# npit/video-learning-tf

Measured on AMD Instinct MI355X. Metric: clips/sec (16-frame 227x227) LRCN train step, higher is better.
Workload: dtype f32; 1 GPU; LRCN AlexNet(fc6)+LSTM(256) 16-frame 227x227x3 clips, 101 classes, UCF-101-shaped synthetic, full train step; global_batch=64, clips_per_gpu=64, frames_per_clip=16, parallelism=dp1, optimizer=sgd+clip_by_global_norm(10), init=reference (sigma 0.05), dist_world_size=1

## Files before the change

### include/vltf.h

```cpp
#ifndef VLTF_H
#define VLTF_H

#include <stddef.h>
#include <stdint.h>

#ifdef __cplusplus
extern "C" {
#endif

typedef void* vl_stream_t;
typedef struct vl_conv_desc vl_conv_desc;

typedef struct vl_step_state {
    int64_t step;
    float lr;
    uint32_t tag_origin;
    float adam_lr;
    uint32_t reserved[3];
} vl_step_state;

const char* vl_last_error(void);
int vl_version(void);
int vl_device_count(void);

int vl_input_prep_u8(const uint8_t* src, float* dst, int n, int raw_h, int raw_w, int out_h, int out_w,
                     const int32_t* crop_y, const int32_t* crop_x, const uint8_t* mirror,
                     const float* mean_bgr, int dst_halo, int dst_phase, vl_stream_t stream);
int vl_nhwc_to_nchw(const float* src, float* dst, int n, int h, int w, int c, int dst_halo, int dst_phase, vl_stream_t stream);
int vl_nchw_to_nhwc(const float* src, float* dst, int n, int c, int h, int w, vl_stream_t stream);

int vl_conv_create(vl_conv_desc** out, int cin, int h, int w, int cout, int kh, int kw, int stride, int groups);
void vl_conv_destroy(vl_conv_desc* d);
int vl_conv_out_hw(const vl_conv_desc* d, int* oh, int* ow);
int vl_conv_set_halo(vl_conv_desc* d, int x_halo, int y_halo, int dy_halo, int dx_halo);
int vl_conv_set_x_phase_split(vl_conv_desc* d, int on);
int vl_conv_x_phase(const vl_conv_desc* d);
int vl_set_conv_math(int math);
int vl_conv_math(void);
int vl_conv_set_row_classes(int on);
int vl_conv_fwd(const vl_conv_desc* d, const float* x, const float* w_hwio, const float* bias, float* y,
                int n, int relu, vl_stream_t stream);
int vl_conv_wt_transpose(const vl_conv_desc* d, const float* w_hwio, float* wt, vl_stream_t stream);
int vl_conv_dgrad(const vl_conv_desc* d, const float* dy, const float* wt, float* dx, const float* relu_mask,
                  int n, vl_stream_t stream);
size_t vl_conv_wgrad_ws_bytes(const vl_conv_desc* d, int n);
int vl_conv_wgrad_fuses_bias(const vl_conv_desc* d);
int vl_conv_wgrad(const vl_conv_desc* d, const float* x, const float* dy, float* dw, float* db, void* ws,
                  size_t ws_bytes, int n, vl_stream_t stream);
size_t vl_c8_bytes(int n, int c, int h, int w, int halo);
int vl_pack_c8(const float* x, void* xb, int n, int c, int h, int w, int x_halo, int xb_halo, vl_stream_t stream);
size_t vl_conv_c8_w_bytes(const vl_conv_desc* d, int bwd);
int vl_conv_c8_pack_w(const vl_conv_desc* d, const float* w_hwio, void* wb, int bwd, vl_stream_t stream);
int vl_conv_c8_fwd(vl_conv_desc* d, const void* xb, const void* wb, const float* bias, float* y, void* yb, int n, int relu,
                   vl_stream_t stream);
int vl_conv_c8_dgrad(vl_conv_desc* d, const void* dyb, const void* wbt, float* dx, void* dxb, const float* relu_mask,
                     const void* relu_mask_c8, int n, vl_stream_t stream);
size_t vl_conv_c8_wgrad_ws_bytes(const vl_conv_desc* d, int n);
int vl_conv_c8_wgrad(vl_conv_desc* d, const void* xb, const void* dyb, float* dw, void* ws, size_t ws_bytes, int n,
                     vl_stream_t stream);
int vl_bias_grad_c8(const void* dyb, float* db, float* ws, int n, int c, int h, int w, int halo, vl_stream_t stream);
int vl_pack_kc8(const float* src, void* dst, int64_t positions, int channels, int64_t pos_stride, int64_t ch_stride, vl_stream_t stream);
size_t vl_gemm_kc8_ws_bytes(int m, int n, int k);
int vl_gemm_kc8(const void* a_kc8, const void* b_kc8, float* c, int m, int n, int k, const float* bias, int relu, void* ws,
                size_t ws_bytes, vl_stream_t stream);
int vl_s2d_c8_from_x0(const vl_conv_desc* d, const float* x0, void* xb, int n, vl_stream_t stream);
int vl_input_prep_u8_s2d(const vl_conv_desc* d, const uint8_t* src, void* xb, int n, int raw_h, int raw_w, const int32_t* crop_y,
                         const int32_t* crop_x, const uint8_t* mirror, const float* mean_bgr, vl_stream_t stream);
int vl_s2d_weights(const vl_conv_desc* d, const float* src, float* dst, int grad, vl_stream_t stream);
int vl_bias_grad_nchw(const float* dy, float* db, float* ws, int n, int c, int hw, vl_stream_t stream);

int vl_lrn_fwd(const float* x, float* y, int n, int c, int hw, int radius, float alpha, float beta, float bias,
               vl_stream_t stream);
// ... 109 lines not shown
```

### video-learning-tf_amd/_ffi.py

```python
import ctypes as C
import os

_HERE = os.path.dirname(os.path.abspath(__file__))
LIB_PATH = os.environ.get("VLTF_HIP_LIB") or os.path.join(_HERE, "libvltf_hip.so")

p = C.c_void_p
i32, i64, f32, u32, u64, sz = C.c_int, C.c_int64, C.c_float, C.c_uint32, C.c_uint64, C.c_size_t

SIGNATURES = {
    "vl_last_error": (C.c_char_p, []),
    "vl_version": (i32, []),
    "vl_device_count": (i32, []),
    "vl_input_prep_u8": (i32, [p, p, i32, i32, i32, i32, i32, p, p, p, p, i32, i32, p]),
    "vl_nhwc_to_nchw": (i32, [p, p, i32, i32, i32, i32, i32, i32, p]),
    "vl_nchw_to_nhwc": (i32, [p, p, i32, i32, i32, i32, p]),
    "vl_conv_create": (i32, [C.POINTER(p), i32, i32, i32, i32, i32, i32, i32, i32]),
    "vl_conv_destroy": (None, [p]),
    "vl_conv_out_hw": (i32, [p, C.POINTER(i32), C.POINTER(i32)]),
    "vl_conv_set_halo": (i32, [p, i32, i32, i32, i32]),
    "vl_conv_set_x_phase_split": (i32, [p, i32]),
    "vl_conv_x_phase": (i32, [p]),
    "vl_set_conv_math": (i32, [i32]),
    "vl_conv_math": (i32, []),
    "vl_conv_set_row_classes": (i32, [i32]),
    "vl_gemm_split_ws_bytes": (C.c_size_t, [i32, i32, i32]),
    "vl_conv_fwd": (i32, [p, p, p, p, p, i32, i32, p]),
    "vl_conv_wt_transpose": (i32, [p, p, p, p]),
    "vl_conv_dgrad": (i32, [p, p, p, p, p, i32, p]),
    "vl_conv_wgrad_ws_bytes": (sz, [p, i32]),
    "vl_conv_wgrad_fuses_bias": (i32, [p]),
    "vl_conv_wgrad": (i32, [p, p, p, p, p, p, sz, i32, p]),
    "vl_c8_bytes": (sz, [i32, i32, i32, i32, i32]),
    "vl_pack_c8": (i32, [p, p, i32, i32, i32, i32, i32, i32, p]),
    "vl_conv_c8_w_bytes": (sz, [p, i32]),
    "vl_conv_c8_pack_w": (i32, [p, p, p, i32, p]),
    "vl_conv_c8_fwd": (i32, [p, p, p, p, p, p, i32, i32, p]),
    "vl_conv_c8_dgrad": (i32, [p, p, p, p, p, p, p, i32, p]),
    "vl_pack_kc8": (i32, [p, p, i64, i32, i64, i64, p]),
    "vl_gemm_kc8_ws_bytes": (sz, [i32, i32, i32]),
    "vl_gemm_kc8": (i32, [p, p, p, i32, i32, i32, p, i32, p, sz, p]),
    "vl_s2d_c8_from_x0": (i32, [p, p, p, i32, p]),
    "vl_input_prep_u8_s2d": (i32, [p, p, p, i32, i32, i32, p, p, p, p, p]),
    "vl_s2d_weights": (i32, [p, p, p, i32, p]),
    "vl_bias_grad_c8": (i32, [p, p, p, i32, i32, i32, i32, i32, p]),
    "vl_conv_c8_wgrad_ws_bytes": (sz, [p, i32]),
    "vl_conv_c8_wgrad": (i32, [p, p, p, p, p, sz, i32, p]),
    "vl_bias_grad_nchw": (i32, [p, p, p, i32, i32, i32, p]),
    "vl_lrn_fwd": (i32, [p, p, i32, i32, i32, i32, f32, f32, f32, p]),
    "vl_lrn_bwd": (i32, [p, p, p, i32, i32, i32, i32, f32, f32, f32, i32, i32, i32, p]),
    "vl_lrn_pool_fwd": (i32, [p, p, p, i32, i32, i32, i32, i32, i32, f32, f32, f32, p]),
    "vl_pool_lrn_bwd": (i32, [p, p, p, p, i32, i32, i32, i32, i32, i32, f32, f32, f32, i32, i32, p]),
    "vl_pool_lrn_bwd_test_ranges": (i32, [i32]),
    "vl_lrn_pool_fwd_c8": (i32, [p, i32, p, p, i32, i32, i32, i32, i32, i32, f32, f32, f32, p]),
    "vl_pool_lrn_bwd_c8": (i32, [p, i32, p, p, p, i32, i32, i32, i32, i32, i32, f32, f32, f32, i32, i32, p]),
    "vl_maxpool_fwd": (i32, [p, p, p, i32, i32, i32, i32, i32, i32, i64, i64, i64, i64, p]),
    "vl_maxpool_bwd": (i32, [p, p, p, p, i32, i32, i32, i32, i32, i32, i64, i64, i64, i64, i32, p]),
    "vl_gemm": (i32, [i32, i32, i32, i32, i32, p, i64, p, i64, p, i64, p, i32, p, p, sz, p]),
# ... 88 lines not shown
```

### video-learning-tf_amd/csrc/conv_desc.h

```cpp
#pragma once
#include <hip/hip_runtime.h>
#include <stdint.h>

struct vl_conv_rowcls {
    int ncls;
    int oh0[5];
    int rows[5];
    int K[5];
    int tab0[5];
    int rt0[5];
};

struct vl_conv_desc {
    int cin, h, w, cout, kh, kw, stride, groups;
    int oh, ow, pt, pl, pb, pr;
    int cig, cog;
    int K;
    int Kd;
    int x_halo, y_halo, dy_halo, dx_halo;
    int x_phase;
    int2* ktab2_fwd;
    int* ktab_fwd;
    int2* ptab2_fwd;
    int2* ptab2_bwd;
    int* ptab_fwd;
    int* ptab_bwd;
    int* rowtab_fwd;
    int* rowtab_bwd;
    int fwd_padded, bwd_padded;
    vl_conv_rowcls rc_fwd, rc_bwd;
    uint32_t* wsplit_fwd;
    uint32_t* wsplit_bwd;
    int* c8_toff_fwd;
    int* c8_toff_bwd;
};

void conv_c8_free_tables(vl_conv_desc* d);
int conv_c8_build_tables(vl_conv_desc* d);
```

### video-learning-tf_amd/csrc/mfma_gemm.hip

```cpp
#include <stdlib.h>
#include <string.h>

#include "common.h"
#include "conv_desc.h"

typedef float f32x16 __attribute__((ext_vector_type(16)));
typedef const __attribute__((address_space(4))) int* const_int_ptr;
__device__ __forceinline__ const_int_ptr as_const(const int* p) { return (const_int_ptr)(uintptr_t)p; }
static constexpr int NT = 256;
static constexpr int KBLK = 16;

static constexpr uint32_t OOB_OFF = 0xF0000000u;
static constexpr int64_t MAX_BUF_BYTES = 0xE0000000ll;

__device__ __forceinline__ __amdgpu_buffer_rsrc_t make_rsrc(const float* base, int64_t bytes) {
    return __builtin_amdgcn_make_buffer_rsrc(const_cast<float*>(base), 0, (int)(uint32_t)bytes, 0x00020000);
}
__device__ __forceinline__ float buf_load(__amdgpu_buffer_rsrc_t r, uint32_t voff, int soff) {
    return __builtin_bit_cast(float, __builtin_amdgcn_raw_buffer_load_b32(r, (int)voff, soff, 0));
}

template <int BX, int BR>
struct LdsTile {
    static constexpr int STR = BR + 2;
// ... 557 lines not shown

template <int I> struct IntC { static constexpr int value = I; };
template <int B, int E, typename F>
__device__ __forceinline__ void static_for(F&& f) {
    if constexpr (B < E) {
        f(IntC<B>{});
        static_for<B + 1, E>(f);
    }
}
struct SplitBf16 {
    i32x4 p[3];
};
template <int NPC>
__device__ __forceinline__ void split_pieces(float x0, float x1, int (&out)[3]) {
    f32x2 r = {x0, x1};
#pragma unroll
    for (int k = 0; k < NPC; ++k) {
        const uint32_t h = __builtin_bit_cast(uint32_t, __builtin_convertvector(r, bf16x2));
        out[k] = (int)h;
        if (k + 1 < NPC) r = f32x2{r[0] - __uint_as_float(h << 16), r[1] - __uint_as_float(h & 0xffff0000u)};
    }
}
__device__ constexpr int kProdA[6] = {0, 0, 1, 1, 0, 2};
__device__ constexpr int kProdB[6] = {0, 1, 0, 1, 2, 0};
constexpr int split_products(int math) { return math == 6 ? 6 : math == 3 ? 3 : 1; }
constexpr int split_pieces_of(int math) { return math == 6 ? 3 : math == 3 ? 2 : 1; }
__device__ __forceinline__ f32x16 mfma_bf16(const i32x4& a, const i32x4& b, const f32x16& c) {
    return __builtin_amdgcn_mfma_f32_32x32x16_bf16(__builtin_bit_cast(bf16x8, a), __builtin_bit_cast(bf16x8, b), c, 0, 0, 0);
}

template <int BN, int WM, int WN, int MATH = 0, bool X4 = false>
__global__ __launch_bounds__(NT, 1) void wgrad_dma_kernel(const ConvGeom g, const DyParams d, const EpiRowMajor::Params pe,
                                                          int tiles_i, int tiles_j, int groups, int units, int rtiles,
                                                          int rt_per_split, float* db_slabs, int db_stride) {
    using C = WgradDmaCfg<BN>;
    constexpr int BM = C::BM, STR = C::STR, SA = BM * STR, BUF = C::BUF;
    constexpr int TM = BM / WM / 32, TN = BN / WN / 32;
    constexpr int RA = BM / 4, RB = BN / 4;
    static_assert(WM * WN == 4 && TM * WM * 32 == BM && TN * WN * 32 == BN, "tile shape");
    static_assert(RA + RB <= 10 * 2 * TM * TN, "row fetches must leave the last third of a tile's MFMAs to cover their latency");
    static_assert(!X4 || (MATH != 0 && BN == 128 && BM == 128), "the 16-byte fetch form: split-product modes, 128 x 128 tiles");
    constexpr int GSTR = 258, SA4 = 32 * GSTR, BUF4 = 64 * GSTR;
    extern __shared__ __attribute__((aligned(16))) float ldsw[];

    const int tiles = tiles_i * tiles_j;
    const int k8 = blockIdx.x >> 3;
    const int unit = (k8 / tiles) * 8 + (blockIdx.x & 7);
    if (unit >= units) return;
    const int tile_id = k8 % tiles;
    const int ti_blk = tile_id % tiles_i, tj_blk = tile_id / tiles_i;
    const int zg = unit % groups, zs = unit / groups;
    const int i0 = ti_blk * BM, j0 = tj_blk * BN;
    const int lane = threadIdx.x & 63;
    const int wave = __builtin_amdgcn_readfirstlane(threadIdx.x >> 6);
    const int wi0 = (wave / WN) * (BM / WM), wj0 = (wave % WN) * (BN / WN);

    const i32x4 rs_x = rsrc_words(g.x + (int64_t)zg * g.grp_stride, (g.total - (int64_t)zg * g.grp_stride) * 4);
    const int64_t goff = (int64_t)zg * d.Cog * d.plane;
    const i32x4 rs_dy = rsrc_words(d.dy + goff, (d.total - goff) * 4);
    const int* tab = g.ktab + i0 + wave * RA;
    const uint32_t lds0 = (uint32_t)(uintptr_t)(__attribute__((address_space(3))) float*)ldsw;
    const int row_bytes = (int)(d.plane * 4);
    const int b_row0 = j0 + wave * RB;
    const int b_last = d.Cog - 1;
    const int64_t dy_img = (int64_t)d.Cout_total * d.plane;

    uint32_t voff_x, voff_dy;
    auto decode = [&](int rt) __attribute__((always_inline)) {
        const int m = X4 ? rt * 64 + 4 * (lane & 15) : rt * 64 + lane;
        const bool vm = m < g.M;
        const uint32_t mm = vm ? m : 0;
        const uint32_t n = fd_div(mm, g.dOHW);
        const uint32_t p = mm - n * g.OHW;
        const uint32_t oh = fd_div(p, g.dOW);
        const uint32_t ow = p - oh * g.OW;
        const int ih0 = (int)oh * g.stride - g.pt + g.halo, iw0 = (int)ow * g.col_mul + g.col_add;
        const uint32_t vx = (uint32_t)((int64_t)n * g.img_stride + (int64_t)ih0 * g.Wp + iw0) * 4u;
        const uint32_t vd = (uint32_t)((int64_t)n * dy_img + (int64_t)(oh + d.halo) * d.OWp + ow + d.halo) * 4u;
        voff_x = vm ? vx : OOB_OFF;
        voff_dy = vm ? vd : OOB_OFF;
        asm volatile("" : "+v"(voff_x), "+v"(voff_dy));
    };
    int tabv[RA];
    auto load_table = [&](int rt) __attribute__((always_inline)) {
        const const_int_ptr tt = (const_int_ptr)(uintptr_t)(tab + rt * g.zero);
#pragma unroll
        for (int f = 0; f < RA; ++f) tabv[f] = tt[f];
    };
    auto pin_table = [&]() __attribute__((always_inline)) {
#pragma unroll
        for (int f = 0; f < RA; ++f) asm volatile("" : "+s"(tabv[f]));
    };
    auto dma = [&](const int nb, const int f, int rt_next) __attribute__((always_inline)) {
        const int z = rt_next * g.zero;
        if (f < RA) {
            const uint32_t la = lds0 + (uint32_t)(wave * (RA * STR) + z) * 4u;
            lds_dma_row(rs_x, la + (uint32_t)(nb * BUF + f * STR) * 4u, voff_x, tabv[f]);
        } else {
            const int r = f - RA;
            const uint32_t lb = lds0 + (uint32_t)(SA + wave * (RB * STR) + z) * 4u;
            lds_dma_row(rs_dy, lb + (uint32_t)(nb * BUF + r * STR) * 4u, voff_dy, min(b_row0 + z + r, b_last) * row_bytes);
        }
    };
    uint32_t vrow_a[8], vrow_b[8];
    if constexpr (X4) {
#pragma unroll
        for (int j = 0; j < 8; ++j) {
            const int rl = wave * 8 + j + 32 * (lane >> 4);
            vrow_a[j] = i0 + rl < g.K ? (uint32_t)g.ktab[i0 + rl] : OOB_OFF;
            vrow_b[j] = j0 + rl < d.Cog ? (uint32_t)(j0 + rl) * (uint32_t)row_bytes : OOB_OFF;
        }
    }
    auto dma_x4 = [&](const int nb, const int f, int rt_next) __attribute__((always_inline)) {
        const int z = rt_next * g.zero;
        if (f < 8) {
            const uint32_t vo = (vrow_a[f] == OOB_OFF || voff_x == OOB_OFF) ? OOB_OFF : vrow_a[f] + voff_x;
            lds_dma_row4(rs_x, lds0 + (uint32_t)(nb * BUF4 + (wave * 8 + f) * GSTR + z) * 4u, vo, 0);
        } else {
            const uint32_t vo = (vrow_b[f - 8] == OOB_OFF || voff_dy == OOB_OFF) ? OOB_OFF : vrow_b[f - 8] + voff_dy;
            lds_dma_row4(rs_dy, lds0 + (uint32_t)(nb * BUF4 + SA4 + (wave * 8 + f - 8) * GSTR + z) * 4u, vo, 0);
        }
    };
    const int ones_row = (db_slabs != nullptr && g.K >= i0 && g.K < i0 + BM) ? g.K - i0 : -1;
    auto finish_tile = [&](const int nb) __attribute__((always_inline)) {
        asm volatile("s_waitcnt vmcnt(0)" ::: "memory");
        if constexpr (X4) {
            if (ones_row >= 0 && ((ones_row & 31) >> 3) == wave) ldsw[nb * BUF4 + (ones_row & 31) * GSTR + (ones_row >> 5) * 64 + lane] = 1.0f;
        } else {
            if (ones_row >= 0 && (ones_row / RA) == wave) ldsw[nb * BUF + ones_row * STR + lane] = 1.0f;
        }
        __syncthreads();
    };

    f32x16 acc[TM][TN];
#pragma unroll
    for (int a = 0; a < TM; ++a)
#pragma unroll
        for (int b = 0; b < TN; ++b)
#pragma unroll
            for (int q = 0; q < 16; ++q) acc[a][b][q] = 0.f;

    const int rt0 = zs * rt_per_split;
    const int rt1 = min(rtiles, rt0 + rt_per_split);
    const int ntiles = rt1 - rt0;
    if (ntiles > 0) {
        decode(rt0);
        load_table(rt0);
        pin_table();
        if constexpr (X4) {
#pragma unroll
            for (int f = 0; f < 16; ++f) dma_x4(0, f, rt0);
        } else {
#pragma unroll
            for (int f = 0; f < RA + RB; ++f) dma(0, f, rt0);
        }
        decode(rt0 + 1);
        finish_tile(0);
    }
    const float* fa = ldsw + (wi0 + (lane & 31)) * STR + 2 * (lane >> 5);
    const float* fb = ldsw + SA + (wj0 + (lane & 31)) * STR + 2 * (lane >> 5);

    auto tile = [&](const int cur, int rt_next) __attribute__((always_inline)) {
        float2 af[2][TM], bf[2][TN];
#pragma unroll
        for (int a = 0; a < TM; ++a) af[0][a] = *reinterpret_cast<const float2*>(fa + cur * BUF + a * 32 * STR);
#pragma unroll
        for (int b = 0; b < TN; ++b) bf[0][b] = *reinterpret_cast<const float2*>(fb + cur * BUF + b * 32 * STR);
#pragma unroll
        for (int t = 0; t < 16; ++t) {
            const int c = t & 1, nx = c ^ 1;
            if (t + 1 < 16) {
#pragma unroll
                for (int a = 0; a < TM; ++a) af[nx][a] = *reinterpret_cast<const float2*>(fa + cur * BUF + a * 32 * STR + 4 * (t + 1));
#pragma unroll
                for (int b = 0; b < TN; ++b) bf[nx][b] = *reinterpret_cast<const float2*>(fb + cur * BUF + b * 32 * STR + 4 * (t + 1));
            }
#pragma unroll
            for (int m = 0; m < 2 * TM * TN; ++m) {
                const int a = (m % (TM * TN)) / TN, b = m % TN;
                if (m < TM * TN) acc[a][b] = __builtin_amdgcn_mfma_f32_32x32x2f32(af[c][a].x, bf[c][b].x, acc[a][b], 0, 0, 0);
                else acc[a][b] = __builtin_amdgcn_mfma_f32_32x32x2f32(af[c][a].y, bf[c][b].y, acc[a][b], 0, 0, 0);
                const int f = t * (2 * TM * TN) + m;
                if (f < RA + RB) {
                    dma(cur ^ 1, f, rt_next);
                    __builtin_amdgcn_sched_barrier(0);
                }
            }
            if (t == 10) {
                load_table(rt_next + 1);
                __builtin_amdgcn_sched_barrier(0);
            }
            if (t == 13) {
                int rtn = rt_next + 1;
                asm volatile("" : "+s"(rtn));
                decode(rtn);
                pin_table();
                __builtin_amdgcn_sched_barrier(0);
            }
        }
        finish_tile(cur ^ 1);
    };
    const float* fa3 = ldsw + (wi0 + (lane & 31)) * STR + 8 * (lane >> 5);
    const float* fb3 = ldsw + SA + (wj0 + (lane & 31)) * STR + 8 * (lane >> 5);
    auto tile_split = [&](const int cur, int rt_next) __attribute__((always_inline)) {
        constexpr int NP = split_products(MATH), NPC = split_pieces_of(MATH);
        constexpr int NMS = NP * TM * TN, NTOT = 4 * NMS, NF = X4 ? 16 : RA + RB;
        constexpr int FSPAN = NTOT >= 28 ? NTOT - 14 : NTOT / 2;
        constexpr int FPM = (NF + FSPAN - 1) / FSPAN, FEND = (NF + FPM - 1) / FPM;
        constexpr int LT = FEND > NTOT - 12 ? FEND : NTOT - 12;
        constexpr int PIN = LT + 2 > NTOT - 6 ? LT + 2 : NTOT - 6;
        static_assert(PIN < NTOT, "the tile must leave room to load and pin the next table");
        SplitBf16 As[2][TM], Bs[2][TN];
        auto load_split = [&](const int st, SplitBf16 (&A)[TM], SplitBf16 (&B)[TN]) __attribute__((always_inline)) {
#pragma unroll
            for (int a = 0; a < TM; ++a)
#pragma unroll
                for (int q = 0; q < 4; ++q) {
                    const float2 v = X4 ? *reinterpret_cast<const float2*>(ldsw + cur * BUF4 + (lane & 31) * GSTR + (wi0 / 32 + a) * 64 + 16 * st +
                                                                            8 * (lane >> 5) + 2 * q)
                                        : *reinterpret_cast<const float2*>(fa3 + cur * BUF + a * 32 * STR + 16 * st + 2 * q);
                    int pc[3] = {0, 0, 0};
                    split_pieces<NPC>(v.x, v.y, pc);
#pragma unroll
                    for (int k = 0; k < NPC; ++k) A[a].p[k][q] = pc[k];
                }
#pragma unroll
            for (int b = 0; b < TN; ++b)
#pragma unroll
                for (int q = 0; q < 4; ++q) {
                    const float2 v = X4 ? *reinterpret_cast<const float2*>(ldsw + cur * BUF4 + SA4 + (lane & 31) * GSTR + (wj0 / 32 + b) * 64 +
                                                                            16 * st + 8 * (lane >> 5) + 2 * q)
                                        : *reinterpret_cast<const float2*>(fb3 + cur * BUF + b * 32 * STR + 16 * st + 2 * q);
                    int pc[3] = {0, 0, 0};
// ... 9 lines not shown
            static_for<0, NMS>([&](auto MI) __attribute__((always_inline)) {
                constexpr int m = decltype(MI)::value;
                constexpr int prod = m / (TM * TN), a = (m % (TM * TN)) / TN, b = m % TN;
                acc[a][b] = mfma_bf16(As[c][a].p[kProdA[prod]], Bs[c][b].p[kProdB[prod]], acc[a][b]);
                constexpr int idx = st * NMS + m;
                static_for<0, FPM>([&](auto EI) __attribute__((always_inline)) {
                    constexpr int f = idx * FPM + decltype(EI)::value;
                    if constexpr (f < NF) {
                        if constexpr (X4) dma_x4(cur ^ 1, f, rt_next);
                        else dma(cur ^ 1, f, rt_next);
                    }
                });
                __builtin_amdgcn_sched_barrier(0x106);
                if constexpr (idx == LT) load_table(rt_next + 1);
                if constexpr (idx == PIN) {
                    int rtn = rt_next + 1;
                    asm volatile("" : "+s"(rtn));
                    decode(rtn);
                    pin_table();
                }
            });
        });
        finish_tile(cur ^ 1);
    };
    auto run_tile = [&](const int cur, int rt_next) __attribute__((always_inline)) {
        if constexpr (MATH != 0) tile_split(cur, rt_next);
        else tile(cur, rt_next);
    };
    int rt = rt0;
    for (int i = 0; i + 1 < ntiles; i += 2, rt += 2) {
        run_tile(0, rt + 1);
        run_tile(1, rt + 2);
    }
    if (ntiles > 0 && (ntiles & 1)) run_tile(0, rt + 1);

    EpiRowMajor::template apply<TM, TN>(pe, zg, zs, i0 + wi0, j0 + wj0, acc);
    if (ones_row >= 0) {
        float* dbs = db_slabs + (int64_t)zs * db_stride + zg * d.Cog;
        const int lr = ones_row - wi0;
        if (lr >= 0 && lr < BM / WM) {
            const int a = lr >> 5, rr = lr & 31;
            const int q = (rr & 3) + 4 * (rr >> 3);
            if (((rr >> 2) & 1) == (lane >> 5)) {
#pragma unroll
                for (int b = 0; b < TN; ++b) {
                    const int j = j0 + wj0 + 32 * b + (lane & 31);
                    float v = 0.f;
#pragma unroll
                    for (int aa = 0; aa < TM; ++aa)
#pragma unroll
                        for (int qq = 0; qq < 16; ++qq)
                            if (aa == a && qq == q) v = acc[aa][b][qq];
                    if (j < d.Cog) dbs[j] = v;
                }
            }
        }
    }
}

typedef float f32x4 __attribute__((ext_vector_type(4)));
typedef float f32x4u __attribute__((ext_vector_type(4), aligned(4)));

struct ConvDmaParams {
    const float* w;
    int64_t w_ld;
    int64_t w_grp_stride;
    int64_t w_bytes;
// ... 798 lines not shown
        const int blocks = (int)((count + 255) / 256 < 4096 ? (count + 255) / 256 : 4096);
        hipLaunchKernelGGL(reduce_slabs_kernel<1>, dim3(blocks), dim3(256), 0, s, ws, out, count, splits, slab_stride, bias, ncols, ldc, relu, mask);
    }
}

static const bool kConvStaged = vl_exp_env("VL_CONV_STAGED") != nullptr;
static const bool kGemmNoSplit = vl_exp_env("VL_GEMM_NOSPLIT") != nullptr;
static const bool kConvNoWideStore = vl_exp_env("VL_CONV_NO_WIDE_STORE") != nullptr;
static const bool kConvNoTailSplit = vl_exp_env("VL_CONV_NO_TAIL_SPLIT") != nullptr;
static const bool kConvNoLoadPick = vl_exp_env("VL_CONV_NO_LOAD_PICK") != nullptr;
static const bool kWgradDword = vl_exp_env("VL_WGRAD_DWORD") != nullptr;
static const bool kRing8 = vl_exp_env("VL_CONV_RING8") != nullptr;

static int g_conv_math = [] {
    const char* e = vl_exp_env("VL_CONV_MATH");
    return e == nullptr ? 0 : strcmp(e, "bf16x3") == 0 ? 3 : strcmp(e, "bf16x6") == 0 ? 6 : strcmp(e, "bf16") == 0 ? 1 : 0;
}();

extern "C" int vl_set_conv_math(int math) {
    VL_CHECK(math == 0 || math == 1 || math == 3 || math == 6, "vl_set_conv_math: 0 (fp32), 1 (bf16), 3 (bf16x3) or 6 (bf16x6)");
    g_conv_math = math;
    return 0;
}

extern "C" int vl_conv_math(void) { return g_conv_math; }

static int g_conv_row_classes = 1;

extern "C" int vl_conv_set_row_classes(int on) {
    g_conv_row_classes = on ? 1 : 0;
    return 0;
}


static void tf_same_pad(int in, int k, int s, int* out, int* before, int* after) {
    *out = (in + s - 1) / s;
    int total = (*out - 1) * s + k - in;
    if (total < 0) total = 0;
    *before = total / 2;
    *after = total - *before;
}


static void k_to_row(int k, int kh, int kw, int cg, bool permuted, int* ky, int* kx, int* c) {
    if (permuted) {
        const int cl = k % KBLK, t = k / KBLK;
        *kx = t % kw;
        *ky = (t / kw) % kh;
        *c = (t / (kw * kh)) * KBLK + cl;
    } else {
        *c = k % cg;
        *kx = (k / cg) % kw;
        *ky = k / (cg * kw);
    }
}

static void free_dev(void* p) {
    if (p) (void)hipFree(p);
}

template <class T>
static int upload(T** dev, const T* host, size_t count) {
    free_dev(*dev);
    *dev = nullptr;
    hipError_t e = hipMalloc((void**)dev, sizeof(T) * count);
    if (e == hipSuccess) e = hipMemcpy(*dev, host, sizeof(T) * count, hipMemcpyHostToDevice);
// ... 62 lines not shown
            }
        for (int i = 0; i < ncls; ++i) {
            const int c = order[i], Kc = (c_hi[c] - c_lo[c] + 1) * kw * cg;
            rc->oh0[i] = c_oh0[c]; rc->rows[i] = c_rows[c]; rc->K[i] = Kc;
            if (Kc == K) {
                rc->tab0[i] = 0; rc->rt0[i] = 0;
                continue;
            }
            rc->tab0[i] = (int)n1; rc->rt0[i] = (int)n3;
            int kc = 0;
            for (int k = 0; k < K; ++k) {
                int ky, kx, ch;
                k_to_row(k, kh, kw, cg, true, &ky, &kx, &ch);
                if (ky < c_lo[c] || ky > c_hi[c]) continue;
                h1[n1 + kc] = h1[k];
                if (kc % KBLK == 0) h3[n3 + kc / KBLK] = h3[k / KBLK];
                ++kc;
            }
            n1 += ((Kc + 127) / 128) * 128 + 256;
            n3 += (((Kc + 127) / 128) * 128 + 256) / KBLK;
        }
        rc->ncls = ncls;
    }
    int rcode = upload(dev1, h1, n1);
    if (rcode == 0) rcode = upload(dev2, h2, pad);
    if (rcode == 0 && rowtab) rcode = upload(rowtab, h3, n3);
    if (rcode && rc) rc->ncls = 0;
    free(h1);
    free(h2);
    free(h3);
    return rcode;
}

static int rebuild_tables(vl_conv_desc* d) {
    d->fwd_padded = d->x_halo >= d->pt && d->x_halo >= d->pb && d->x_halo >= d->pl && d->x_halo >= d->pr;
    if (!d->fwd_padded) d->x_phase = 1;
    const int ph = d->x_phase > 1 ? d->x_phase : 1, shift = d->x_halo - d->pl;
    int rc = build_ktabs(&d->ktab_fwd, &d->ktab2_fwd, nullptr, d->kh, d->kw, d->cig, d->h, d->w, d->x_halo, false, ph, shift);
    if (rc == 0)
        rc = build_ktabs(&d->ptab_fwd, &d->ptab2_fwd, &d->rowtab_fwd, d->kh, d->kw, d->cig, d->h, d->w, d->x_halo, d->cig % KBLK == 0, ph,
                         shift, d->stride == 1 ? &d->rc_fwd : nullptr, d->pt, d->oh);
    if (rc == 0 && d->stride == 1) {
        rc = build_ktabs(&d->ptab_bwd, &d->ptab2_bwd, &d->rowtab_bwd, d->kh, d->kw, d->cog, d->oh, d->ow, d->dy_halo, d->cog % KBLK == 0, 1,
                         0, &d->rc_bwd, d->kh - 1 - d->pt, d->h);
        const int need = (d->kh - 1 - d->pt > d->pt ? d->kh - 1 - d->pt : d->pt);
        const int needw = (d->kw - 1 - d->pl > d->pl ? d->kw - 1 - d->pl : d->pl);
        d->bwd_padded = d->dy_halo >= need && d->dy_halo >= needw;
    }
    if (rc == 0) rc = conv_c8_build_tables(d);
    return rc;
}

extern "C" int vl_conv_create(vl_conv_desc** out, int cin, int h, int w, int cout, int kh, int kw, int stride, int groups) {
    VL_CHECK(out, "vl_conv_create: null out");
    VL_CHECK(cin > 0 && cout > 0 && h > 0 && w > 0 && kh > 0 && kw > 0 && stride > 0 && groups > 0, "vl_conv_create: bad geometry");
    VL_CHECK(cin % groups == 0 && cout % groups == 0, "vl_conv_create: channels not divisible by groups");
    VL_CHECK(h < 0x4000 && w < 0x4000 && kh < 256 && kw < 256, "vl_conv_create: plane too large");
    vl_conv_desc* d = (vl_conv_desc*)calloc(1, sizeof(vl_conv_desc));
    VL_CHECK(d, "vl_conv_create: out of host memory");
    d->cin = cin; d->h = h; d->w = w; d->cout = cout; d->kh = kh; d->kw = kw; d->stride = stride; d->groups = groups;
    tf_same_pad(h, kh, stride, &d->oh, &d->pt, &d->pb);
    tf_same_pad(w, kw, stride, &d->ow, &d->pl, &d->pr);
    d->cig = cin / groups;
    d->cog = cout / groups;
    d->K = kh * kw * d->cig;
    d->Kd = kh * kw * d->cog;
    const size_t sf = (size_t)groups * ceil_div(d->K, KBLK) * 24 * (ceil_div(d->cog, 128) * 128) * 4;
    const size_t sb = (size_t)groups * ceil_div(d->Kd, KBLK) * 24 * (ceil_div(d->cig, 128) * 128) * 4;
    const bool images = sf <= (64u << 20) && sb <= (64u << 20);
    if (rebuild_tables(d) || (images && (hipMalloc((void**)&d->wsplit_fwd, sf) != hipSuccess || hipMalloc((void**)&d->wsplit_bwd, sb) != hipSuccess))) {
        vl_conv_destroy(d);
        vl_set_error("vl_conv_create: device table allocation failed");
        return 2;
    }
    *out = d;
    return 0;
}

extern "C" int vl_conv_set_halo(vl_conv_desc* d, int x_halo, int y_halo, int dy_halo, int dx_halo) {
    VL_CHECK(d, "vl_conv_set_halo: null descriptor");
    VL_CHECK(x_halo >= 0 && y_halo >= 0 && dy_halo >= 0 && dx_halo >= 0 && x_halo < 64 && y_halo < 64 && dy_halo < 64 && dx_halo < 64,
             "vl_conv_set_halo: bad halo");
    d->x_halo = x_halo; d->y_halo = y_halo; d->dy_halo = dy_halo; d->dx_halo = dx_halo;
    VL_CHECK(rebuild_tables(d) == 0, "vl_conv_set_halo: device table allocation failed");
    return 0;
}

extern "C" int vl_conv_set_x_phase_split(vl_conv_desc* d, int on) {
    VL_CHECK(d, "vl_conv_set_x_phase_split: null descriptor");
    VL_CHECK(!on || d->fwd_padded, "vl_conv_set_x_phase_split: needs the padded x layout (set the halo first)");
    d->x_phase = (on && d->stride > 1) ? d->stride : 1;
    VL_CHECK(rebuild_tables(d) == 0, "vl_conv_set_x_phase_split: device table allocation failed");
    return 0;
}

extern "C" int vl_conv_x_phase(const vl_conv_desc* d) { return d && d->x_phase > 1 ? d->x_phase : 1; }

extern "C" void vl_conv_destroy(vl_conv_desc* d) {
    if (!d) return;
    free_dev(d->ktab_fwd);
    free_dev(d->ktab2_fwd);
    free_dev(d->ptab_fwd);
    free_dev(d->ptab2_fwd);
    free_dev(d->ptab_bwd);
    free_dev(d->ptab2_bwd);
    free_dev(d->rowtab_fwd);
    free_dev(d->rowtab_bwd);
    free_dev(d->wsplit_fwd);
    free_dev(d->wsplit_bwd);
    conv_c8_free_tables(d);
    free(d);
}

extern "C" int vl_conv_out_hw(const vl_conv_desc* d, int* oh, int* ow) {
    VL_CHECK(d, "vl_conv_out_hw: null descriptor");
    if (oh) *oh = d->oh;
    if (ow) *ow = d->ow;
    return 0;
}

struct ConvOut {
    float* y;
    const float* bias;
    const float* mask;
    int relu;
    int y_halo, m_halo, OH, OW;
};

template <int BM, int WM, int WN, bool PADDED>
static int launch_conv(const ConvGeom& g, const float* w, int64_t w_ld, int w_grp_stride, const int* row_tab, int Cog,
                       int Cout_total, const ConvOut& o, hipStream_t s) {
    constexpr int BN = 128, BR = KBLK;
    using LA = ConvWeightKX<BM, BR>;
    using LB = ConvGather<BN, BR, PADDED>;
    typename LA::Params pa{w, w_ld, Cog, g.K, (int64_t)w_grp_stride, row_tab};
    EpiConvNCHW::Params pe;
    pe.y = o.y; pe.bias = o.bias; pe.mask = o.mask; pe.relu = o.relu;
    pe.Cog = Cog; pe.Cout_total = Cout_total; pe.OHW = g.OHW; pe.OW = g.OW; pe.M = g.M;
    pe.dOHW = g.dOHW; pe.dOW = g.dOW;
    pe.y_halo = o.y_halo; pe.y_wp = o.OW + 2 * o.y_halo; pe.y_plane = (int64_t)(o.OH + 2 * o.y_halo) * pe.y_wp;
// ... 534 lines not shown
                       ceil_div(rtiles, splits));
    VL_LAUNCH_CHECK();
    return reduce_wgrad(d, dw, ws, splits, s);
}

template <int BN, int WM, int WN>
static int launch_wgrad_dma(const vl_conv_desc* d, const ConvGeom& g, const float* dy, float* dw, float* db, float* ws, int splits,
                            hipStream_t s) {
    using C = WgradDmaCfg<BN>;
    DyParams pb;
    dy_params(d, g, dy, pb);
    const int64_t slab = (int64_t)d->K * d->cout;
    EpiRowMajor::Params pe{splits > 1 ? ws : dw, d->cout, d->K, d->cog, nullptr, nullptr, 0, d->cog, splits > 1 ? slab : 0};
    const int tiles_i = ceil_div(d->K, C::BM), tiles_j = ceil_div(d->cog, BN);
    const int rtiles = ceil_div(g.M, C::BR);
    static bool attr_set[8] = {false, false, false, false, false, false, false, false};
    int v = g_conv_math == 6 ? 3 : g_conv_math == 3 ? 2 : g_conv_math == 1 ? 1 : 0;
    auto kern = v == 3 ? wgrad_dma_kernel<BN, WM, WN, 6> : v == 2 ? wgrad_dma_kernel<BN, WM, WN, 3>
              : v == 1 ? wgrad_dma_kernel<BN, WM, WN, 1> : wgrad_dma_kernel<BN, WM, WN, 0>;
    if constexpr (BN == 128) {
        if (v != 0 && g.OW % 4 == 0 && g.col_mul == 1 && !kWgradDword) {
            kern = v == 3 ? wgrad_dma_kernel<BN, WM, WN, 6, true> : v == 2 ? wgrad_dma_kernel<BN, WM, WN, 3, true> : wgrad_dma_kernel<BN, WM, WN, 1, true>;
            v += 4;
        }
    }
    if (!attr_set[v]) {
        VL_HIP(hipFuncSetAttribute(reinterpret_cast<const void*>(kern), hipFuncAttributeMaxDynamicSharedMemorySize, (int)C::LDS_BYTES));
        attr_set[v] = true;
    }
    float* db_slabs = db ? (splits > 1 ? ws + (int64_t)splits * slab : db) : nullptr;
    const int units = d->groups * splits;
    dim3 grid((unsigned)(ceil_div(units, 8) * 8 * tiles_i * tiles_j), 1, 1);
    hipLaunchKernelGGL(kern, grid, dim3(NT), C::LDS_BYTES, s, g, pb, pe, tiles_i, tiles_j, d->groups, units, rtiles,
                       ceil_div(rtiles, splits), db_slabs, d->cout);
    VL_LAUNCH_CHECK();
    if (db && splits > 1) {
        launch_reduce_slabs(s, db_slabs, db, (int64_t)d->cout, splits, (int64_t)d->cout, nullptr, 0, 0, 0, nullptr);
        VL_LAUNCH_CHECK();
    }
    return reduce_wgrad(d, dw, ws, splits, s);
}

static int device_cus() {
    static int cus = 0;
    if (!cus) {
        int dev = 0;
        hipDeviceProp_t p;
        if (hipGetDevice(&dev) == hipSuccess && hipGetDeviceProperties(&p, dev) == hipSuccess) cus = p.multiProcessorCount;
        if (cus <= 0) cus = 256;
    }
    return cus;
}

static int wgrad_splits(const vl_conv_desc* d, int n) {
    const int64_t M = (int64_t)n * d->oh * d->ow;
    const int tiles = ceil_div(d->K, 128) * ceil_div(d->cog, d->cog % 128 == 0 ? 128 : 96) * d->groups;
    if (!d->fwd_padded) {
        const int rtiles = ceil_div(M, 32);
        int splits = ceil_div(2048, tiles);
        return splits > rtiles ? rtiles : (splits < 1 ? 1 : splits);
    }
    const int rtiles = ceil_div(M, 64);
    static const int forced = vl_exp_env("VL_WGRAD_SPLITS") ? atoi(vl_exp_env("VL_WGRAD_SPLITS")) : 0;
    if (forced >= 1 && forced <= rtiles) return forced;
    const int per_xcd = device_cus() / 8 > 0 ? device_cus() / 8 : 1;
    const int64_t slab_bytes = ((int64_t)d->K + 1) * d->cout * 4;
    int best = 1;
// ... 333 lines not shown
```

### video-learning-tf_amd/ops.py

```python
import ctypes as C

import torch

from . import _ffi

F32 = torch.float32


def stream():
    return torch.cuda.current_stream().cuda_stream


def _p(t):
    return None if t is None else t.data_ptr()


def _f32(*ts):
    for t in ts:
        if t is None:
            continue
        if not (t.is_cuda and t.dtype == F32):
            raise _ffi.VltfError("expected a CUDA/HIP float32 tensor, got %s on %s" % (t.dtype, t.device))


# ... 578 lines not shown
              stream())


def step_guard(skip, *lstm_workspaces):
    _skip_word(skip)
    first = True
    for ws in lstm_workspaces:
        if ws is not None:
            _ffi.call("vl_status_or", _p(skip), _p(ws), int(first), stream())
            first = False
    return skip


def fill(t, value):
    _f32(t)
    _ffi.call("vl_fill", _p(t), t.numel(), value, stream())


CONV_MATH = {"f32": 0, "bf16": 1, "bf16x3": 3, "bf16x6": 6}


def set_conv_math(name):
    if name not in CONV_MATH:
        raise _ffi.VltfError("conv math must be one of %s, not %r" % (sorted(CONV_MATH), name))
    _ffi.call("vl_set_conv_math", CONV_MATH[name])


def conv_math():
    return {v: k for k, v in CONV_MATH.items()}[int(_ffi.lib().vl_conv_math())]


def conv_set_row_classes(on=True):
    _ffi.call("vl_conv_set_row_classes", int(bool(on)))


def relu_grad(d, y, count=None):
    _f32(d, y); _dense(d, y)
    _ffi.call("vl_relu_grad", _p(d), _p(y), d.numel() if count is None else int(count), stream())


def copy2d(src, dst, rows, cols, src_ld=None, dst_ld=None):
    _f32(src, dst)
    _ffi.call("vl_copy2d", _p(src), cols if src_ld is None else int(src_ld), _p(dst), cols if dst_ld is None else int(dst_ld),
              int(rows), int(cols), stream())


ELTWISE_OP = {"add": 0, "avg": 1, "maximum": 2}


def eltwise2(a, b, out, op, count=None):
    _f32(a, b, out)
    _ffi.call("vl_eltwise2", _p(a), _p(b), _p(out), a.numel() if count is None else int(count), ELTWISE_OP[op], stream())


def max2_grad(a, b, d, da, db, count=None):
    _f32(a, b, d, da, db)
    _ffi.call("vl_max2_grad", _p(a), _p(b), _p(d), _p(da), _p(db), a.numel() if count is None else int(count), stream())


FUSE_OP = {"avg": 0, "maximum": 1}


def _ptr_list(ts):
    arr = (C.c_void_p * len(ts))()
    for i, t in enumerate(ts):
        arr[i] = None if t is None else t.data_ptr()
# ... 56 lines not shown
```

Baseline: 1906 clips/s.

## Skip MFMA k-steps in conv wgrad for padding-only output windows

Precomputes, for each 128-row weight-gradient tile of padded stride-1 convolutions, the output-pixel window that can touch real input. In the f32 wgrad DMA kernel, a wave ballot marks 4-pixel k-steps whose pixels all fall outside that window, and inline-asm branches skip those MFMA groups. Padded taps then stop doing zero multiplies at border pixels. The cost is extra scalar branching, hand-written asm with manual nops, and accumulator fences before the epilogue. The path is on by default and only applies in the plain f32 math mode.

```diff
diff --git a/include/vltf.h b/include/vltf.h
--- a/include/vltf.h
+++ b/include/vltf.h
@@ -38,6 +38,7 @@
 int vl_set_conv_math(int math);
 int vl_conv_math(void);
 int vl_conv_set_row_classes(int on);
+int vl_conv_set_wgrad_skip(int on);
 int vl_conv_fwd(const vl_conv_desc* d, const float* x, const float* w_hwio, const float* bias, float* y,
                 int n, int relu, vl_stream_t stream);
 int vl_conv_wt_transpose(const vl_conv_desc* d, const float* w_hwio, float* wt, vl_stream_t stream);
diff --git a/video-learning-tf_amd/_ffi.py b/video-learning-tf_amd/_ffi.py
--- a/video-learning-tf_amd/_ffi.py
+++ b/video-learning-tf_amd/_ffi.py
@@ -23,6 +23,7 @@
     "vl_set_conv_math": (i32, [i32]),
     "vl_conv_math": (i32, []),
     "vl_conv_set_row_classes": (i32, [i32]),
+    "vl_conv_set_wgrad_skip": (i32, [i32]),
     "vl_gemm_split_ws_bytes": (C.c_size_t, [i32, i32, i32]),
     "vl_conv_fwd": (i32, [p, p, p, p, p, i32, i32, p]),
     "vl_conv_wt_transpose": (i32, [p, p, p, p]),
diff --git a/video-learning-tf_amd/csrc/conv_desc.h b/video-learning-tf_amd/csrc/conv_desc.h
--- a/video-learning-tf_amd/csrc/conv_desc.h
+++ b/video-learning-tf_amd/csrc/conv_desc.h
@@ -27,6 +27,7 @@
     int* ptab_bwd;
     int* rowtab_fwd;
     int* rowtab_bwd;
+    int* wgrad_win;
     int fwd_padded, bwd_padded;
     vl_conv_rowcls rc_fwd, rc_bwd;
     uint32_t* wsplit_fwd;
diff --git a/video-learning-tf_amd/csrc/mfma_gemm.hip b/video-learning-tf_amd/csrc/mfma_gemm.hip
--- a/video-learning-tf_amd/csrc/mfma_gemm.hip
+++ b/video-learning-tf_amd/csrc/mfma_gemm.hip
@@ -613,8 +613,9 @@
 template <int BN, int WM, int WN, int MATH = 0, bool X4 = false>
 __global__ __launch_bounds__(NT, 1) void wgrad_dma_kernel(const ConvGeom g, const DyParams d, const EpiRowMajor::Params pe,
                                                           int tiles_i, int tiles_j, int groups, int units, int rtiles,
-                                                          int rt_per_split, float* db_slabs, int db_stride) {
+                                                          int rt_per_split, float* db_slabs, int db_stride, const int* win) {
     using C = WgradDmaCfg<BN>;
+    constexpr bool SKIP = MATH == 0 && !X4;
     constexpr int BM = C::BM, STR = C::STR, SA = BM * STR, BUF = C::BUF;
     constexpr int TM = BM / WM / 32, TN = BN / WN / 32;
     constexpr int RA = BM / 4, RB = BN / 4;
@@ -646,6 +647,16 @@
     const int b_last = d.Cog - 1;
     const int64_t dy_img = (int64_t)d.Cout_total * d.plane;
 
+    uint32_t w_oh_lo = 0, w_oh_span = 0, w_ow_lo = 0, w_ow_span = 0, w_on = 0;
+    if constexpr (SKIP) {
+        if (win != nullptr) {
+            const const_int_ptr wp = (const_int_ptr)(uintptr_t)(win + 4 * ti_blk);
+            w_oh_lo = (uint32_t)wp[0]; w_oh_span = (uint32_t)wp[1]; w_ow_lo = (uint32_t)wp[2]; w_ow_span = (uint32_t)wp[3];
+            w_on = wp[1] >= 0 ? 1u : 0u;
+        }
+        asm volatile("" : "+v"(w_oh_lo), "+v"(w_oh_span), "+v"(w_ow_lo), "+v"(w_ow_span), "+v"(w_on));
+    }
+    uint64_t skipq = 0;
     uint32_t voff_x, voff_dy;
     auto decode = [&](int rt) __attribute__((always_inline)) {
         const int m = X4 ? rt * 64 + 4 * (lane & 15) : rt * 64 + lane;
@@ -661,6 +672,18 @@
         voff_x = vm ? vx : OOB_OFF;
         voff_dy = vm ? vd : OOB_OFF;
         asm volatile("" : "+v"(voff_x), "+v"(voff_dy));
+        if constexpr (SKIP) {
+            const bool outside = !vm || oh - w_oh_lo > w_oh_span || ow - w_ow_lo > w_ow_span;
+            uint64_t b = __builtin_amdgcn_ballot_w64(outside && w_on != 0);
+            b &= b >> 1;
+            b &= b >> 2;
+            b &= 0x1111111111111111ull;
+            b = (b | b >> 3) & 0x0303030303030303ull;
+            b = (b | b >> 6) & 0x000f000f000f000full;
+            b = (b | b >> 12) & 0x000000ff000000ffull;
+            b = (b | b >> 24) & 0xffffull;
+            skipq = (skipq & 0xffffffffull) | b << 32;
+        }
     };
     int tabv[RA];
     auto load_table = [&](int rt) __attribute__((always_inline)) {
@@ -726,6 +749,7 @@
     const int ntiles = rt1 - rt0;
     if (ntiles > 0) {
         decode(rt0);
+        skipq >>= 16;
         load_table(rt0);
         pin_table();
         if constexpr (X4) {
@@ -736,50 +760,88 @@
             for (int f = 0; f < RA + RB; ++f) dma(0, f, rt0);
         }
         decode(rt0 + 1);
+        skipq >>= 16;
         finish_tile(0);
     }
     const float* fa = ldsw + (wi0 + (lane & 31)) * STR + 2 * (lane >> 5);
     const float* fb = ldsw + SA + (wj0 + (lane & 31)) * STR + 2 * (lane >> 5);
 
+    auto mfma1 = [](f32x16& cacc, float x, float y, uint64_t sq, auto T, bool first) __attribute__((always_inline)) {
+        constexpr int t = decltype(T)::value;
+        if (first) asm volatile("s_nop 1\n\ts_bitcmp1_b64 %3, %4\n\ts_cbranch_scc1 1f\n\tv_mfma_f32_32x32x2_f32 %0, %1, %2, %0\n1:"
+                                : "+a"(cacc) : "v"(x), "v"(y), "s"(sq), "n"(t) : "scc");
+        else asm volatile("s_bitcmp1_b64 %3, %4\n\ts_cbranch_scc1 1f\n\tv_mfma_f32_32x32x2_f32 %0, %1, %2, %0\n1:"
+                          : "+a"(cacc) : "v"(x), "v"(y), "s"(sq), "n"(t) : "scc");
+    };
+    auto mfma_step = [](f32x16 (&cacc)[TM][TN], const float2 (&A)[TM], const float2 (&B)[TN], uint64_t sq, auto T) __attribute__((always_inline)) {
+        constexpr int t = decltype(T)::value;
+        if constexpr (TM == 2 && TN == 2) {
+            asm volatile("s_bitcmp1_b64 %12, %13\n\ts_cbranch_scc1 1f\n\t"
+                         "v_mfma_f32_32x32x2_f32 %0, %4, %8, %0\n\tv_mfma_f32_32x32x2_f32 %1, %4, %10, %1\n\t"
+                         "v_mfma_f32_32x32x2_f32 %2, %6, %8, %2\n\tv_mfma_f32_32x32x2_f32 %3, %6, %10, %3\n\t"
+                         "v_mfma_f32_32x32x2_f32 %0, %5, %9, %0\n\tv_mfma_f32_32x32x2_f32 %1, %5, %11, %1\n\t"
+                         "v_mfma_f32_32x32x2_f32 %2, %7, %9, %2\n\tv_mfma_f32_32x32x2_f32 %3, %7, %11, %3\n1:"
+                         : "+a"(cacc[0][0]), "+a"(cacc[0][1]), "+a"(cacc[1][0]), "+a"(cacc[1][1])
+                         : "v"(A[0].x), "v"(A[0].y), "v"(A[1].x), "v"(A[1].y), "v"(B[0].x), "v"(B[0].y), "v"(B[1].x), "v"(B[1].y), "s"(sq), "n"(t)
+                         : "scc");
+        } else {
+            static_assert(TM == 1 && TN == 3, "mfma_step: wave tile shapes of launch_wgrad_dma");
+            asm volatile("s_bitcmp1_b64 %11, %12\n\ts_cbranch_scc1 1f\n\t"
+                         "v_mfma_f32_32x32x2_f32 %0, %3, %5, %0\n\tv_mfma_f32_32x32x2_f32 %1, %3, %7, %1\n\tv_mfma_f32_32x32x2_f32 %2, %3, %9, %2\n\t"
+                         "v_mfma_f32_32x32x2_f32 %0, %4, %6, %0\n\tv_mfma_f32_32x32x2_f32 %1, %4, %8, %1\n\tv_mfma_f32_32x32x2_f32 %2, %4, %10, %2\n1:"
+                         : "+a"(cacc[0][0]), "+a"(cacc[0][1]), "+a"(cacc[0][2])
+                         : "v"(A[0].x), "v"(A[0].y), "v"(B[0].x), "v"(B[0].y), "v"(B[1].x), "v"(B[1].y), "v"(B[2].x), "v"(B[2].y), "s"(sq), "n"(t)
+                         : "scc");
+        }
+    };
+    auto acc_fence = [&]() __attribute__((always_inline)) {
+#pragma unroll
+        for (int k = 0; k < TM * TN; ++k) asm volatile("s_nop 7\n\ts_nop 7\n\ts_nop 7" : "+a"(acc[k / TN][k % TN]));
+    };
     auto tile = [&](const int cur, int rt_next) __attribute__((always_inline)) {
         float2 af[2][TM], bf[2][TN];
 #pragma unroll
         for (int a = 0; a < TM; ++a) af[0][a] = *reinterpret_cast<const float2*>(fa + cur * BUF + a * 32 * STR);
 #pragma unroll
         for (int b = 0; b < TN; ++b) bf[0][b] = *reinterpret_cast<const float2*>(fb + cur * BUF + b * 32 * STR);
-#pragma unroll
-        for (int t = 0; t < 16; ++t) {
-            const int c = t & 1, nx = c ^ 1;
-            if (t + 1 < 16) {
+        static_for<0, 16>([&](auto T) __attribute__((always_inline)) {
+            constexpr int t = decltype(T)::value;
+            constexpr int c = t & 1, nx = c ^ 1;
+            if constexpr (t + 1 < 16) {
 #pragma unroll
                 for (int a = 0; a < TM; ++a) af[nx][a] = *reinterpret_cast<const float2*>(fa + cur * BUF + a * 32 * STR + 4 * (t + 1));
 #pragma unroll
                 for (int b = 0; b < TN; ++b) bf[nx][b] = *reinterpret_cast<const float2*>(fb + cur * BUF + b * 32 * STR + 4 * (t + 1));
             }
-#pragma unroll
-            for (int m = 0; m < 2 * TM * TN; ++m) {
-                const int a = (m % (TM * TN)) / TN, b = m % TN;
-                if (m < TM * TN) acc[a][b] = __builtin_amdgcn_mfma_f32_32x32x2f32(af[c][a].x, bf[c][b].x, acc[a][b], 0, 0, 0);
-                else acc[a][b] = __builtin_amdgcn_mfma_f32_32x32x2f32(af[c][a].y, bf[c][b].y, acc[a][b], 0, 0, 0);
-                const int f = t * (2 * TM * TN) + m;
-                if (f < RA + RB) {
-                    dma(cur ^ 1, f, rt_next);
-                    __builtin_amdgcn_sched_barrier(0);
+            if constexpr (t * (2 * TM * TN) < RA + RB) {
+#pragma unroll
+                for (int m = 0; m < 2 * TM * TN; ++m) {
+                    const int a = (m % (TM * TN)) / TN, b = m % TN;
+                    if (m < TM * TN) mfma1(acc[a][b], af[c][a].x, bf[c][b].x, skipq, T, t == 0 && m == 0);
+                    else mfma1(acc[a][b], af[c][a].y, bf[c][b].y, skipq, T, false);
+                    const int f = t * (2 * TM * TN) + m;
+                    if (f < RA + RB) {
+                        dma(cur ^ 1, f, rt_next);
+                        __builtin_amdgcn_sched_barrier(0);
+                    }
                 }
-            }
-            if (t == 10) {
+            } else {
+                mfma_step(acc, af[c], bf[c], skipq, T);
+            }
+            if constexpr (t == 10) {
                 load_table(rt_next + 1);
                 __builtin_amdgcn_sched_barrier(0);
             }
-            if (t == 13) {
+            if constexpr (t == 13) {
                 int rtn = rt_next + 1;
                 asm volatile("" : "+s"(rtn));
                 decode(rtn);
                 pin_table();
                 __builtin_amdgcn_sched_barrier(0);
             }
-        }
+        });
         finish_tile(cur ^ 1);
+        skipq >>= 16;
     };
     const float* fa3 = ldsw + (wi0 + (lane & 31)) * STR + 8 * (lane >> 5);
     const float* fb3 = ldsw + SA + (wj0 + (lane & 31)) * STR + 8 * (lane >> 5);
@@ -855,7 +917,11 @@
         run_tile(0, rt + 1);
         run_tile(1, rt + 2);
     }
-    if (ntiles > 0 && (ntiles & 1)) run_tile(0, rt + 1);
+    if constexpr (SKIP) acc_fence();
+    if (ntiles > 0 && (ntiles & 1)) {
+        run_tile(0, rt + 1);
+        if constexpr (SKIP) acc_fence();
+    }
 
     EpiRowMajor::template apply<TM, TN>(pe, zg, zs, i0 + wi0, j0 + wj0, acc);
     if (ones_row >= 0) {
@@ -1720,6 +1786,13 @@
     return 0;
 }
 
+static int g_wgrad_skip = 1;
+
+extern "C" int vl_conv_set_wgrad_skip(int on) {
+    g_wgrad_skip = on ? 1 : 0;
+    return 0;
+}
+
 
 static void tf_same_pad(int in, int k, int s, int* out, int* before, int* after) {
     *out = (in + s - 1) / s;
@@ -1848,6 +1921,31 @@
     return rcode;
 }
 
+static int build_wgrad_windows(vl_conv_desc* d) {
+    free_dev(d->wgrad_win);
+    d->wgrad_win = nullptr;
+    if (d->stride != 1 || d->kh <= 1 || !d->fwd_padded) return 0;
+    const int nt = ceil_div(d->K, 128);
+    int* hw = (int*)malloc(sizeof(int) * 4 * nt);
+    if (!hw) return 1;
+    for (int ti = 0; ti < nt; ++ti) {
+        const int r0 = ti * 128, r1 = (r0 + 128 < d->K ? r0 + 128 : d->K) - 1;
+        const int tap0 = r0 / d->cig, tap1 = r1 / d->cig;
+        const int ky0 = tap0 / d->kw, ky1 = tap1 / d->kw;
+        const int kx0 = ky0 == ky1 ? tap0 % d->kw : 0, kx1 = ky0 == ky1 ? tap1 % d->kw : d->kw - 1;
+        const int oh_lo = d->pt - ky1 > 0 ? d->pt - ky1 : 0, oh_hi = d->h - 1 + d->pt - ky0 < d->oh - 1 ? d->h - 1 + d->pt - ky0 : d->oh - 1;
+        const int ow_lo = d->pl - kx1 > 0 ? d->pl - kx1 : 0, ow_hi = d->w - 1 + d->pl - kx0 < d->ow - 1 ? d->w - 1 + d->pl - kx0 : d->ow - 1;
+        const bool never = (d->K % 128 != 0 && ti == nt - 1) || oh_lo > oh_hi || ow_lo > ow_hi;
+        hw[4 * ti + 0] = oh_lo;
+        hw[4 * ti + 1] = never ? -1 : oh_hi - oh_lo;
+        hw[4 * ti + 2] = ow_lo;
+        hw[4 * ti + 3] = never ? 0 : ow_hi - ow_lo;
+    }
+    const int rcode = upload(&d->wgrad_win, hw, (size_t)4 * nt);
+    free(hw);
+    return rcode;
+}
+
 static int rebuild_tables(vl_conv_desc* d) {
     d->fwd_padded = d->x_halo >= d->pt && d->x_halo >= d->pb && d->x_halo >= d->pl && d->x_halo >= d->pr;
     if (!d->fwd_padded) d->x_phase = 1;
@@ -1863,6 +1961,7 @@
         const int needw = (d->kw - 1 - d->pl > d->pl ? d->kw - 1 - d->pl : d->pl);
         d->bwd_padded = d->dy_halo >= need && d->dy_halo >= needw;
     }
+    if (rc == 0) rc = build_wgrad_windows(d);
     if (rc == 0) rc = conv_c8_build_tables(d);
     return rc;
 }
@@ -1922,6 +2021,7 @@
     free_dev(d->ptab2_bwd);
     free_dev(d->rowtab_fwd);
     free_dev(d->rowtab_bwd);
+    free_dev(d->wgrad_win);
     free_dev(d->wsplit_fwd);
     free_dev(d->wsplit_bwd);
     conv_c8_free_tables(d);
@@ -2522,7 +2622,7 @@
     const int units = d->groups * splits;
     dim3 grid((unsigned)(ceil_div(units, 8) * 8 * tiles_i * tiles_j), 1, 1);
     hipLaunchKernelGGL(kern, grid, dim3(NT), C::LDS_BYTES, s, g, pb, pe, tiles_i, tiles_j, d->groups, units, rtiles,
-                       ceil_div(rtiles, splits), db_slabs, d->cout);
+                       ceil_div(rtiles, splits), db_slabs, d->cout, g_wgrad_skip ? d->wgrad_win : nullptr);
     VL_LAUNCH_CHECK();
     if (db && splits > 1) {
         launch_reduce_slabs(s, db_slabs, db, (int64_t)d->cout, splits, (int64_t)d->cout, nullptr, 0, 0, 0, nullptr);
diff --git a/video-learning-tf_amd/ops.py b/video-learning-tf_amd/ops.py
--- a/video-learning-tf_amd/ops.py
+++ b/video-learning-tf_amd/ops.py
@@ -634,6 +634,10 @@
 
 def conv_set_row_classes(on=True):
     _ffi.call("vl_conv_set_row_classes", int(bool(on)))
+
+
+def conv_set_wgrad_skip(on=True):
+    _ffi.call("vl_conv_set_wgrad_skip", int(bool(on)))
 
 
 def relu_grad(d, y, count=None):
```

Result: slower. 1884 clips/s (-1.1%).
